# wangxb29/PPST

Hardware: AMD Instinct MI355X
Metric: 512x512 portrait swaps/sec/GPU (higher is better)
Workload: dtype bf16x3 (fp32 split into hi+lo bf16, 3 MFMA passes, fp32 accumulate); 1 GPU; simple_swapping 512x512 batch=8 per GPU, generator+encoders forward only (BASELINE configs[1]); image_parallel=1 batch per rank, no data-path collective

## Files before the change

include/ppst_hip.h:

```cpp
#ifndef PPST_HIP_H
#define PPST_HIP_H

#include <stddef.h>
#include <stdint.h>

#ifdef __cplusplus
extern "C" {
#endif

#define PPST_OK 0
#define PPST_EINVAL (-1)
#define PPST_EUNSUPPORTED (-2)
#define PPST_ENULL (-3)

enum { PPST_F32 = 0, PPST_F16 = 1, PPST_BF16 = 2, PPST_F64 = 3  };

enum { PPST_PAD_ZERO = 0, PPST_PAD_REFLECT = 1, PPST_PAD_REPLICATE = 2 };

enum { PPST_ACT_NONE = 0, PPST_ACT_LRELU = 1 , PPST_ACT_PRELU = 2 };

#define PPST_ABI_VERSION 3
int ppst_version(void);

#define PPST_ST_F32 0
// ... 67 lines not shown
int ppst_upscale_weight(const void* w, void* out, int cout, int cin, float scale, void* stream);
int ppst_dgrad_s2d_stack_weight(const void* w, void* out, int cout, int cin, void* stream);
int ppst_depth_to_space_st(const void* x, void* y, int B, int th, int tw, int oh, int ow, int C, int st, void* stream);

#define PPST_KSPLIT_SCRATCH_BYTES ((size_t)256 * 512 * 128 * 4)
#define PPST_KSPLIT_FLAG_WORDS 4096

typedef struct ppst_conv_args {
  const void* x;
  const void* wpack;
  const void* steps;
  void* y;
  const void* bias;
  const void* noise;
  const void* prelu;
  void* stats;
  const void* residual;
  float noise_weight;
  float out_scale;
  int32_t B, in_h, in_w, in_ld;
  int32_t out_h, out_w, out_ld, cout;
  int32_t nsteps, n_groups;
  int32_t pad_mode;
  int32_t in_off_y, in_off_x;
  int32_t out_sy, out_sx;
  int32_t act;
  int32_t precision;
  int32_t res_ld;
  int32_t tile_h, tile_w;
  int32_t halo;
  int32_t bn;
  const void* in_scale_shift;
  const void* in_prelu;
  int32_t in_c, in_act;
  int32_t flop_steps;
  int32_t tile_rows;
  int32_t a_slots;
  int32_t early_a;
  int32_t variant;
  int32_t in_presplit;
  int32_t dual_b;
  int32_t io_st;
  int32_t k64;
  const void* in_res;
  int32_t in_res_ld;
  int32_t ksplit;
  const int32_t* ksplit_starts;
  void* ksplit_scratch;
  unsigned* ksplit_flags;
  uint32_t ksplit_epoch;
} ppst_conv_args;

int ppst_conv2d_mfma(const ppst_conv_args* a, void* stream);
int64_t ppst_conv_pack_wino_bytes(int cout, int cin);
int ppst_conv_pack_wino(const void* w, int64_t sn, int64_t sc, int64_t sy, int64_t sx, float scale, int cout, int cin,
                        void* out, void* stream);
int ppst_presplit(const void* x, void* y, int64_t npix, int C, int x_ld, int y_ld, void* stream);
int ppst_has_experiments(void);
int ppst_conv2d_f32(const ppst_conv_args* a, const void* w, int64_t sn, int64_t sc, int64_t sy, int64_t sx, float wscale,
                    const int32_t* src_c, const int32_t* src_ky, const int32_t* src_kx, void* stream);
int ppst_conv_tiles(int tile_h, int tile_w, int tile_rows);

int ppst_conv1x1_small_cin(const void* x, const void* w, const void* bias, void* y,
                           int64_t npix, int cin, int in_ld, int cout, float wscale,
                           int act, void* stream);
int ppst_conv1x1_small_cin_st(const void* x, const void* w, const void* bias, void* y,
                              int64_t npix, int cin, int in_ld, int cout, float wscale,
                              int act, int y_st , void* stream);
int ppst_conv1x1_small_cout(const void* x, const void* w, const void* bias, void* y,
                            int64_t npix, int cin, int cout, float wscale, void* stream);
int ppst_conv1x1_small_cout_st(const void* x, const void* w, const void* bias, void* y,
                               int64_t npix, int cin, int cout, float wscale, int x_st , void* stream);
int ppst_torgb_apply_st(const void* x, const void* scale_shift, const void* res, int res_ld, float out_scale, const void* w,
                        const void* bias, void* y, int B, int H, int W, int cin, float wscale, int x_st, void* stream);

int ppst_in_stats(const void* x, void* partial, int B, int H, int W, int C, int ld,
                  int rep_pad, int* n_partials, void* stream);
int ppst_in_finalize(const void* partial, int n_partials, const void* style,
                     int style_ld ,
                     const void* post_bias ,
                     void* scale_shift , int B, int C, double count,
                     float eps, void* stream);
int ppst_affine_act(const void* x, const void* scale_shift, const void* res,
                    const void* res_scale_shift , void* y,
                    int B, int64_t hw, int C, int x_ld, int res_ld, int y_ld,
                    int act , const void* prelu,
                    float out_scale,
                    int res_up2_w ,
                    void* stream);
int ppst_affine_act_st(const void* x, const void* scale_shift, const void* res, const void* res_scale_shift, void* y,
                       int B, int64_t hw, int C, int x_ld, int res_ld, int y_ld, int act, const void* prelu,
                       float out_scale, int res_up2_w, int x_st, int y_st, void* stream);
int ppst_affine_act_stats(const void* x, const void* scale_shift, const void* res,
                          const void* res_scale_shift, void* y, void* partial,
                          int B, int H, int W, int C, int x_ld, int res_ld, int y_ld,
                          int act, const void* prelu, float out_scale, int rep_pad,
                          int res_up2 , void* stream);
int ppst_upsample_nearest2(const void* x, void* y, int B, int H, int W, int C, void* stream);
int ppst_upsample_nearest2_st(const void* x, void* y, int B, int H, int W, int C, int st, void* stream);

int64_t ppst_gap_gmp_ws(int B, int64_t hw, int C);
int ppst_gap_gmp(const void* x, const void* mask, void* out, void* ws, int B, int H, int W,
                 int C, int ld, void* stream);
int ppst_gap_gmp_st(const void* x, const void* mask, void* out, void* ws, int B, int H, int W,
                    int C, int ld, int x_st, void* stream);
int ppst_avgpool(const void* x, void* y, int B, int H, int W, int C, int x_ld, int f,
// ... 158 lines not shown
```

ppst_amd/_lib.py:

```python
import ctypes
import os

import torch

HERE = os.path.dirname(os.path.abspath(__file__))
LIB_PATH = os.environ.get("PPST_HIP_LIB") or os.path.join(HERE, "libppst_hip.so")

if not os.path.exists(LIB_PATH):
    raise ImportError(
        "ppst_amd: %s is missing -- build it with `python -m ppst_amd.build` "
        "(hipcc --offload-arch=gfx950). There is no CPU fallback." % LIB_PATH)

lib = ctypes.CDLL(LIB_PATH)

vp, i32, i64, f32, f64 = ctypes.c_void_p, ctypes.c_int, ctypes.c_int64, ctypes.c_float, ctypes.c_double


class PackJob(ctypes.Structure):
    _fields_ = [("w", vp), ("sn", i64), ("sc", i64), ("sy", i64), ("sx", i64), ("src_c", vp), ("src_ky", vp), ("src_kx", vp),
                ("out", vp), ("total", i64), ("block0", i64), ("scale", f32), ("cout", i32), ("bn", i32), ("nsteps", i32),
                ("n_groups", i32), ("x3", i32), ("f16", i32), ("nblocks", i32), ("dual", i32)]


class UpscaleJob(ctypes.Structure):
    _fields_ = [("w", vp), ("out", vp), ("total", i64), ("block0", i64), ("scale", f32), ("cout", i32), ("cin", i32), ("nblocks", i32)]


class ConvArgs(ctypes.Structure):
    _fields_ = [
        ("x", vp), ("wpack", vp), ("steps", vp), ("y", vp), ("bias", vp), ("noise", vp),
        ("prelu", vp), ("stats", vp), ("residual", vp),
        ("noise_weight", f32), ("out_scale", f32),
        ("B", i32), ("in_h", i32), ("in_w", i32), ("in_ld", i32),
        ("out_h", i32), ("out_w", i32), ("out_ld", i32), ("cout", i32),
        ("nsteps", i32), ("n_groups", i32), ("pad_mode", i32),
        ("in_off_y", i32), ("in_off_x", i32), ("out_sy", i32), ("out_sx", i32),
        ("act", i32), ("precision", i32), ("res_ld", i32), ("tile_h", i32), ("tile_w", i32),
        ("halo", i32), ("bn", i32), ("in_scale_shift", vp), ("in_prelu", vp), ("in_c", i32), ("in_act", i32),
        ("flop_steps", i32), ("tile_rows", i32), ("a_slots", i32), ("early_a", i32), ("variant", i32), ("in_presplit", i32), ("dual_b", i32), ("io_st", i32), ("k64", i32),
        ("in_res", vp), ("in_res_ld", i32), ("ksplit", i32), ("ksplit_starts", vp),
        ("ksplit_scratch", vp), ("ksplit_flags", vp), ("ksplit_epoch", ctypes.c_uint32),
    ]


_SIGS = {
    "ppst_version": (i32, []),
    "ppst_guided_filter_tune": (i32, [i32, i32]),
    "ppst_upfirdn2d": (i32, [vp, vp, vp] + [i32] * 14 + [i32, vp]),
    "ppst_blur_nhwc": (i32, [vp, vp, vp] + [i32] * 10 + [vp, i32, vp]),
    "ppst_blur_nhwc_st": (i32, [vp, vp, vp] + [i32] * 10 + [vp, i32, i32, vp]),
    "ppst_fused_bias_act": (i32, [vp, vp, vp, vp, i64, i32, i32, i32, i32, f32, f32, i32, vp]),
    "ppst_nchw_to_nhwc": (i32, [vp, vp, i32, i32, i32, i32, vp]),
    "ppst_nhwc_to_nchw": (i32, [vp, vp, i32, i32, i32, i32, vp]),
    "ppst_conv_pack": (i32, [vp, i64, i64, i64, i64, f32, i32, i32, vp, vp, vp, i32, i32, i32, vp, vp]),
    "ppst_conv_pack_k64": (i32, [vp, i64, i64, i64, i64, f32, i32, i32, vp, vp, vp, i32, i32, i32, i32, vp, vp]),
    "ppst_conv_pack_up9_bytes": (i64, [i32, i32]),
    "ppst_conv_pack_up9": (i32, [vp, i64, i64, i64, i64, f32, i32, i32, vp, vp]),
    "ppst_conv_pack_wino_bytes": (i64, [i32, i32]),
    "ppst_conv_pack_wino": (i32, [vp, i64, i64, i64, i64, f32, i32, i32, vp, vp]),
    "ppst_conv_pack_dual": (i32, [vp, i64, i64, i64, i64, f32, i32, vp, vp, vp, i32, i32, i32, vp, vp]),
    "ppst_upscale_weight": (i32, [vp, vp, i32, i32, f32, vp]),
    "ppst_dgrad_s2d_stack_weight": (i32, [vp, vp, i32, i32, vp]),
    "ppst_depth_to_space_st": (i32, [vp, vp, i32, i32, i32, i32, i32, i32, i32, vp]),
    "ppst_pack_job_blocks": (i32, [i64]),
    "ppst_conv_pack_batch": (i32, [vp, i32, i32, vp]),
    "ppst_upscale_weight_batch": (i32, [vp, i32, i32, vp]),
    "ppst_conv2d_mfma": (i32, [ctypes.POINTER(ConvArgs), vp]),
    "ppst_has_experiments": (i32, []),
    "ppst_presplit": (i32, [vp, vp, i64, i32, i32, i32, vp]),
    "ppst_conv2d_f32": (i32, [ctypes.POINTER(ConvArgs), vp, i64, i64, i64, i64, f32, vp, vp, vp, vp]),
    "ppst_conv_tiles": (i32, [i32, i32, i32]),
    "ppst_conv1x1_small_cin": (i32, [vp, vp, vp, vp, i64, i32, i32, i32, f32, i32, vp]),
    "ppst_conv1x1_small_cin_st": (i32, [vp, vp, vp, vp, i64, i32, i32, i32, f32, i32, i32, vp]),
    "ppst_conv1x1_small_cout": (i32, [vp, vp, vp, vp, i64, i32, i32, f32, vp]),
    "ppst_conv1x1_small_cout_st": (i32, [vp, vp, vp, vp, i64, i32, i32, f32, i32, vp]),
    "ppst_torgb_apply_st": (i32, [vp, vp, vp, i32, f32, vp, vp, vp, i32, i32, i32, i32, f32, i32, vp]),
    "ppst_in_stats": (i32, [vp, vp, i32, i32, i32, i32, i32, i32, ctypes.POINTER(i32), vp]),
    "ppst_in_finalize": (i32, [vp, i32, vp, i32, vp, vp, i32, i32, f64, f32, vp]),
    "ppst_affine_act": (i32, [vp, vp, vp, vp, vp, i32, i64, i32, i32, i32, i32, i32, vp, f32, i32, vp]),
    "ppst_affine_act_st": (i32, [vp, vp, vp, vp, vp, i32, i64, i32, i32, i32, i32, i32, vp, f32, i32, i32, i32, vp]),
    "ppst_affine_act_stats": (i32, [vp, vp, vp, vp, vp, vp, i32, i32, i32, i32, i32, i32, i32, i32, vp, f32, i32, i32, vp]),
    "ppst_upsample_nearest2": (i32, [vp, vp, i32, i32, i32, i32, vp]),
    "ppst_upsample_nearest2_st": (i32, [vp, vp, i32, i32, i32, i32, i32, vp]),
    "ppst_gap_gmp_ws": (i64, [i32, i64, i32]),
    "ppst_gap_gmp": (i32, [vp, vp, vp, vp, i32, i32, i32, i32, i32, vp]),
    "ppst_gap_gmp_st": (i32, [vp, vp, vp, vp, i32, i32, i32, i32, i32, i32, vp]),
    "ppst_avgpool": (i32, [vp, vp, i32, i32, i32, i32, i32, i32, i32, vp]),
    "ppst_bilinear": (i32, [vp, vp, i32, i32, i32, i32, i32, i32, i32, i32, vp]),
    "ppst_head_tail": (i32, [vp, vp, vp, vp, vp] + [i32] * 10 + [vp]),
    "ppst_maxpool2": (i32, [vp, vp, i32, i32, i32, i32, vp]),
    "ppst_linear": (i32, [vp, vp, vp, vp, i32, i32, i32, f32, f32, i32, i32, vp]),
    "ppst_l2norm_rows": (i32, [vp, vp, i32, i32, f32, i32, vp]),
    "ppst_lerp": (i32, [vp, vp, vp, i64, f32, vp]),
    "ppst_spatial_modulation": (i32, [vp, vp, vp, vp, i32, i64, i32, vp]),
    "ppst_spatial_modulation_st": (i32, [vp, vp, vp, vp, i32, i64, i32, i32, vp]),
    "ppst_rselfcorr": (i32, [vp, vp, i32, i32, i32, i32, i32, vp]),
    "ppst_corr_prep": (i32, [vp, vp, i32, i32, i32, i32, vp]),
    "ppst_gemm_nt_f32": (i32, [vp, vp, vp, i32, i32, i32, i32, f32, vp]),
    "ppst_gemm_nn_f32": (i32, [vp, vp, vp, i32, i32, i32, i32, i32, i32, vp]),
    "ppst_unfold_rows": (i32, [vp, vp, i32, i32, i32, i32, i32, vp]),
    "ppst_unfold_rows_bwd": (i32, [vp, vp, i32, i32, i32, i32, i32, vp]),
    "ppst_gemm_nt_split": (i32, [vp, vp, vp, i32, i32, i32, i32, f32, i32, vp]),
    "ppst_gemm_nn_split": (i32, [vp, vp, vp, i32, i32, i32, i32, i32, i32, i32, vp]),
    "ppst_softmax_rows": (i32, [vp, i64, i32, f32, vp]),
    "ppst_unfold_patches": (i32, [vp, vp, i32, i32, i32, i32, i32, vp]),
    "ppst_fold_patches": (i32, [vp, vp, i32, i32, i32, i32, i32, vp]),
    "ppst_tensor2im_u8": (i32, [vp, vp, i32, i32, i32, i32, vp]),
    "ppst_resample_u8": (i32, [vp, vp, i32, i32, i32, i32, i32, i32, vp, vp, i32, vp]),
    "ppst_u8_to_tensor": (i32, [vp, vp, i32, i32, i32, i32, f32, f32, vp]),
    "ppst_guided_filter_ws": (i64, [i32, i32, i32]),
    "ppst_guided_filter": (i32, [vp, vp, vp, vp, i32, i32, i32, i32, f32, vp, vp]),
    "ppst_smooth_local_affine_ws": (i64, [i32, i32, i32]),
    "ppst_smooth_local_affine": (i32, [vp, vp, vp, vp, vp, i32, i32, i32, i32, i32, f32, f32, vp]),
    "ppst_conv_wgrad_f32": (i32, [vp, vp, vp, vp, vp] + [i32] * 11 + [vp]),
    "ppst_conv_wgrad_bf16x3": (i32, [vp, vp, vp, vp, vp] + [i32] * 11 + [vp]),
    "ppst_conv_wgrad_tr": (i32, [vp, vp, vp, vp, vp, vp, i32, i32, i32, i32, i32, i32, i32, i32, i32, i32, i32, vp]),
    "ppst_conv_wgrad_tr2": (i32, [vp, vp, vp, vp, vp, vp, i32, i32, i32, i32, i32, i32, i32, i32, i32, i32, i32, i32, i32, i32, i32, vp]),
    "ppst_wgrad_scatter": (i32, [vp, vp, vp, vp, vp, i64, i64, i64, i64, i32, i32, i32, f32, i32, vp, vp, i32, i32, vp]),
    "ppst_wgrad_small_cin_ws": (i64, [i64, i32, i32]),
    "ppst_wgrad_small_cin": (i32, [vp, vp, vp, vp, i64, i32, i32, i32, f32, i32, vp]),
# ... 77 lines not shown
```

ppst_amd/build.py:

```python
import os
import subprocess
import sys
from concurrent.futures import ThreadPoolExecutor

HERE = os.path.dirname(os.path.abspath(__file__))
CSRC = os.path.join(HERE, "csrc")
OBJ = os.path.join(HERE, "csrc", "_obj")
LIB = os.path.join(HERE, "libppst_hip.so")
EXPERIMENTS = os.environ.get("PPST_EXPERIMENTS") == "1"
SOURCES = ["upfirdn2d.hip", "fused_bias_act.hip", "elementwise.hip", "linear.hip", "conv_mfma.hip", "conv_mfma2.hip", "conv1x1.hip", "conv_wino.hip", "conv_f32.hip",
           "corr.hip", "guided_filter.hip", "train.hip", "train_g.hip", "imageio.hip", "smooth_filter.hip"] + (["conv_ksplit.hip"] if EXPERIMENTS else [])
FLAGS = ["--offload-arch=gfx950", "-O3", "-fPIC", "-std=c++17", "-Wno-unused-result"] + (["-DPPST_EXPERIMENTS"] if EXPERIMENTS else [])
FILE_FLAGS = {"conv_wino.hip": ["-fno-slp-vectorize"]}
MODE_STAMP = os.path.join(HERE, ".libmode")


def _hipcc():
    for c in (os.environ.get("HIPCC"), "/opt/rocm/bin/hipcc", "hipcc"):
        if c and (os.path.isabs(c) and os.path.exists(c) or not os.path.isabs(c)):
            return c
    return "hipcc"


HEADERS = [os.path.join(CSRC, "common.h"), os.path.join(CSRC, "rscl_common.h"), os.path.join(HERE, "..", "include", "ppst_hip.h")]


def _stale(target, deps):
    return not os.path.exists(target) or any(os.path.getmtime(d) > os.path.getmtime(target) for d in deps)


def _mode():
    return "experiments" if EXPERIMENTS else "production"


def _lib_flavour():
    try:
        return open(MODE_STAMP).read().strip()
    except OSError:
        pass
    if not os.path.exists(LIB):
        return None
    try:
        return "experiments" if b"conv_ksplit_kernel" in open(LIB, "rb").read() else "production"
    except OSError:
        return None


def _mode_changed():
    have = _lib_flavour()
    if have is None:
        return os.path.exists(LIB)
    return have != _mode()


def needs_build():
    return (_mode_changed() or _stale(LIB, [os.path.join(CSRC, s) for s in SOURCES] + HEADERS) or
            any(_stale(os.path.join(OBJ, s.replace(".hip", ".o")), [os.path.join(CSRC, s)]) for s in SOURCES if os.path.isdir(OBJ)))


def build(force=False, verbose=True):
    if not force and not needs_build():
        return LIB
    os.makedirs(OBJ, exist_ok=True)
# ... 30 lines not shown
```

ppst_amd/networks/base_network.py:

```python
import math

import torch
from torch import nn

from .. import ops, weights

SQRT2 = math.sqrt(2.0)
INV_SQRT2 = 1.0 / SQRT2


class _Node(nn.Module):
    """parameter container (no behaviour)."""


def to_nhwc(x):
    if x.dim() != 4:
        raise RuntimeError("expected a 4-D NCHW tensor")
    v = x.permute(0, 2, 3, 1)
    if v.is_contiguous():
        ops._chk(v, "input")
        return v
    return ops.nchw_to_nhwc(x)


# ... 58 lines not shown
        val = build()
        self._cache[key] = (ver, val)
        return val

    def plan(self, wname, kind="conv", scale=1.0):
        w = self.p(wname)
        return self.cached(("plan", wname, kind), [w], lambda: ops.ConvPlan(w, kind=kind, scale=scale))

    def refresh_plans(self):
        plans, keep = [], {}
        for key, (ver, val) in self._cache.items():
            if isinstance(key, tuple) and key and key[0] == "plan" and isinstance(val, ops.ConvPlan) and val.precision != 2 \
                    and val.wparam.data_ptr() == self.p(key[1]).data_ptr():
                plans.append(val)
                keep[key] = (ver, val)
        self._cache.clear()
        if not plans:
            return
        sig = tuple((id(pl), tuple(sorted(map(str, pl._packs)))) for pl in plans)
        hit = self.__dict__.get("_repack")
        if hit is not None and hit[0] == sig:
            ops.run_repack(hit[1])
        else:
            self.__dict__["_repack"] = (sig, ops.repack_plans(plans), plans)
        self._cache.update(keep)

    def print_architecture(self, verbose=False):
        n = sum(p.numel() for p in self.parameters())
        print("[Network %s] Total number of parameters : %.3f M" % (type(self).__name__, n / 1e6))

    def from_rgb(self, x, p, out_dtype=torch.float32):
        w = self.p(p + "Conv.weight")
        return ops.conv1x1_small_cin(x, w, self.p(p + "Act.bias"), 1.0 / math.sqrt(w.shape[1]), ops.ACT_LRELU, out_dtype=out_dtype)

    def _norm_act(self, y, st, count, act_bias=None, act=ops.ACT_NONE, **kw):
        ss = ops.in_finalize(st, count, post_bias=act_bias)
        return ops.affine_act(y, ss, act=act, **kw), ss

    def res_block(self, x, p, blur_pad_mode, norm):
        B, H, W, cin = x.shape
        k = self.p(p + "conv2.Blur.kernel")
        ks = k.shape[0]
        w1, w2, ws = self.p(p + "conv1.Conv.weight"), self.p(p + "conv2.Conv.weight"), self.p(p + "skip.Conv.weight")
        sc1 = 1.0 / math.sqrt(cin * 9)
        scs = 1.0 / math.sqrt(cin)
        conv_pad = ops.PAD_REFLECT if blur_pad_mode == ops.PAD_REFLECT else ops.PAD_ZERO
        pad_c = (ks - 2) + 2
        pad_s = (ks - 2) + 0
        xs, _ = ops.blur_nhwc(x, self.p(p + "skip.Blur.kernel"), (pad_s + 1) // 2, pad_s // 2, ops.PAD_ZERO, down=2)
        if not norm:
            y1 = self.plan(p + "conv1.Conv.weight", scale=sc1)(x, bias=self.p(p + "conv1.Act.bias"), act=ops.ACT_LRELU,
                                                                pad_mode=conv_pad)
            skip = self.plan(p + "skip.Conv.weight", scale=scs)(xs)
            xb, bhw = ops.blur_nhwc(y1, k, (pad_c + 1) // 2, pad_c // 2, blur_pad_mode, s2d=True)
            ohw = ((bhw[0] - 3) // 2 + 1, (bhw[1] - 3) // 2 + 1)
            return self.plan(p + "conv2.Conv.weight", "s2d", sc1)(
                xb, bias=self.p(p + "conv2.Act.bias"), act=ops.ACT_LRELU, residual=skip, res_after_act=True,
                out_scale=INV_SQRT2, out_hw=ohw)
        y1, st1 = self.plan(p + "conv1.Conv.weight", scale=sc1)(x, stats=True, pad_mode=conv_pad)
        ss1 = ops.in_finalize(st1, H * W, post_bias=self.p(p + "conv1.Act.bias"))
        ys, sts = self.plan(p + "skip.Conv.weight", scale=scs)(xs, stats=True)
        xb, bhw = ops.blur_nhwc(y1, k, (pad_c + 1) // 2, pad_c // 2, blur_pad_mode, s2d=True, in_ss=ss1, in_act=ops.ACT_LRELU)
        ohw = ((bhw[0] - 3) // 2 + 1, (bhw[1] - 3) // 2 + 1)
        y2, st2 = self.plan(p + "conv2.Conv.weight", "s2d", sc1)(xb, stats=True, out_hw=ohw)
        cnt = ohw[0] * ohw[1]
        ss_s = ops.in_finalize(sts, cnt)
        ss2 = ops.in_finalize(st2, cnt, post_bias=self.p(p + "conv2.Act.bias"))
        return ops.affine_act(y2, ss2, res=ys, res_scale_shift=ss_s, act=ops.ACT_LRELU, out_scale=INV_SQRT2)
```

ppst_amd/ops.py:

```python
import ctypes
import math
import os
import threading

import torch

from . import _lib
from ._lib import lib, check

PAD_ZERO, PAD_REFLECT, PAD_REPLICATE = 0, 1, 2
ACT_NONE, ACT_LRELU, ACT_PRELU = 0, 1, 2
RES_BEFORE_ACT = 1 << 8

PRECISION = {"value": 0}
TILE_ROWS = {"value": 16}
CONV_VARIANT = {"value": 2}
DUAL_CONVT = {"value": True, "min_blocks": 32}
UP9 = {"value": True, "min_blocks": 64, "min_fill": 0.85}
DIRECT_MAX = {"cout": 64, "nsteps": 40, "cout3x3": 64}
WGRAD_SPLIT = {"blocks": 1024, "min_tiles": 4}
WGRAD_X3 = {"value": True}
STREAM_1X1 = {"value": True}
KSPLIT = {"value": os.environ.get("PPST_KSPLIT", "1") != "0", "max_blocks": 256, "min_steps": 16, "variants": (0, 2, 10)}
KSPLIT_SCRATCH_BYTES = 256 * 512 * 128 * 4
KSPLIT_FLAG_WORDS = 4096
KSPLIT_128 = {"value": False, "min_blocks": 32}
TALL_TILE_128 = {"value": False, "min_blocks": 32}
TALL_TILE_SINGLE = {"value": True, "min_blocks": 64}
K64 = {"value": True}
TILE24_128 = {"value": False, "min_blocks": 32, "max_waste": 0.04}
TWO_BLOCK_128 = {"value": False}
TWO_BLOCK_8ROW = {"value": False, "min_blocks": 64}
BATCH_AWARE = {"value": False, "fill": 192}


class batch_aware:

    def __enter__(self):
        self.prev = BATCH_AWARE["value"]
        BATCH_AWARE["value"] = True

    def __exit__(self, *exc):
        BATCH_AWARE["value"] = self.prev
WINO = {"value": True, "min_blocks": 16, "fill": 0, "ksplit_fill": 64}
FUSE_TAIL = {"value": os.environ.get("PPST_FUSE_TAIL", "1") != "0", "torgb": os.environ.get("PPST_FUSE_TORGB", "0") == "1"}
FAT_MIN_BLOCKS = 32


EXPERIMENTS = bool(lib.ppst_has_experiments())


def _need_experiments(what):
    if not EXPERIMENTS:
        raise RuntimeError("%s is an experiment kernel: rebuild the library with PPST_EXPERIMENTS=1 (python -m ppst_amd.build)" % what)


def set_precision(p):
    assert p in (0, 1, 2, 3, 4)
    if p == 4:
        _need_experiments("precision 4 (two-pass fp16)")
    PRECISION["value"] = p


_raw_stream = getattr(torch._C, "_cuda_getCurrentRawStream", None)
_cur_device = getattr(torch._C, "_cuda_getDevice", None)


def _stream():
    if _raw_stream is not None and _cur_device is not None:
        return ctypes.c_void_p(_raw_stream(_cur_device()))
    return ctypes.c_void_p(torch.cuda.current_stream().cuda_stream)


def _chk(t, name="tensor"):
    if t is None:
        return
    if not isinstance(t, torch.Tensor) or not t.is_cuda:
        raise RuntimeError("%s must be a CUDA (HIP) tensor" % name)
    if t.dtype != torch.float32:
        raise RuntimeError("%s must be float32, got %s" % (name, t.dtype))


def _p(t):
    return None if t is None else ctypes.c_void_p(t.data_ptr())


_ST = {torch.float32: 0, torch.float16: 1, torch.bfloat16: 2}
HALF_STORE = {"value": os.environ.get("PPST_HALF_STORE", "1") != "0"}


def act_dtype():
    if HALF_STORE["value"] and not torch.is_grad_enabled():
        return {1: torch.bfloat16, 3: torch.float16}.get(PRECISION["value"], torch.float32)
    return torch.float32


TRAIN_HALF = {"value": os.environ.get("PPST_TRAIN_HALF", "1") != "0"}

# ... 617 lines not shown
                                                   else self.pack_for(bn))
            steps_t = self.steps_up9 if up9 else self.steps_dual if dual else self.steps
        a.x, a.wpack, a.steps, a.y = _p(x), _p(wp), _p(steps_t), _p(out)
        a.k64 = 1 if k64 else 0
        a.variant = variant
        a.dual_b = 1 if dual else 0
        a.bias, a.noise, a.prelu, a.stats = _p(bias), _p(noise), _p(prelu), _p(st)
        a.residual = _p(residual)
        a.res_ld = _nhwc_ld(residual, "residual", half_ok=True) if residual is not None else 0
        a.io_st = _ST[x.dtype]
        a.noise_weight, a.out_scale = float(noise_weight), float(out_scale)
        a.B, a.in_h, a.in_w, a.in_ld = B, H, W, in_ld
        a.out_h, a.out_w, a.out_ld, a.cout = oh, ow, out_ld, self.cout
        a.nsteps, a.n_groups, a.pad_mode = (self.nsteps // 2 if k64 else self.nsteps), (1 if up9 else 2 if dual else self.n_groups), pad_mode
        a.in_off_y = a.in_off_x = 0
        a.out_sy = a.out_sx = osy
        a.act, a.precision = act | (0x100 if res_after_act else 0), self.precision
        a.tile_h, a.tile_w, a.halo, a.bn, a.tile_rows = th, tw, self.halo, bn, rows
        _chk(in_ss, "in_ss"); _chk(in_prelu, "in_prelu")
        a.in_scale_shift, a.in_prelu, a.in_act = _p(in_ss), _p(in_prelu), in_act
        a.in_c = in_ss.shape[1] if in_ss is not None else 0
        if in_res is not None:
            if variant != 4 or in_ss is None or self.precision != 0 or x.dtype != torch.float32:
                raise RuntimeError("in_res needs a 1x1 plan on the streaming kernel (ops.STREAM_1X1), in_ss, precision 0 and fp32 storage")
            if tuple(in_res.shape) != tuple(x.shape):
                raise RuntimeError("in_res must have the conv input's shape %s, got %s" % (tuple(x.shape), tuple(in_res.shape)))
            a.in_res, a.in_res_ld = _p(in_res), _nhwc_ld(in_res, "in_res")
        a.flop_steps = self.flop_steps
        a.a_slots = min(3, self.chunks_per_group)
        a.early_a = self.early_a
        if presplit:
            _need_experiments("pre-split conv input")
            if variant != 0 or bn != 128 or in_ss is not None or self.nsteps // max(1, self.chunks_per_group) < 4:
                raise RuntimeError("pre-split input: tile kernel (bn 128) plans with chunks of >= 4 steps and no in_ss only")
            a.in_presplit = 1
        ks_S, ks_cuts = self._ksplit(variant, a, self.precision == 2) if (KSPLIT["value"] and BATCH_AWARE["value"]) else (0, None)
        stream = _stream()
        if ks_S:
            ks_arr = (ctypes.c_int32 * (ks_S + 1))(*ks_cuts)
            a.ksplit, a.ksplit_starts = ks_S, ctypes.cast(ks_arr, ctypes.c_void_p)
            a.ksplit_scratch, a.ksplit_flags, a.ksplit_epoch = _ksplit_next(stream)
        if self.precision == 2:
            sn, sc, sy, sx = self.wstrides
            c_, ky_, kx_ = self.src_dev
            check(lib.ppst_conv2d_f32(ctypes.byref(a), _p(self.wsrc), sn, sc, sy, sx, self.scale, _p(c_), _p(ky_), _p(kx_), stream),
                  "ppst_conv2d_f32")
        else:
            check(lib.ppst_conv2d_mfma(ctypes.byref(a), stream), "ppst_conv2d_mfma")
        if stats:
            return out, st
        return out


class _KsWorkspace:
    __slots__ = ("scratch", "flags", "ptrs", "launches")

    def __init__(self):
        self.scratch = torch.empty(KSPLIT_SCRATCH_BYTES, dtype=torch.uint8, device="cuda")
        self.flags = torch.zeros(KSPLIT_FLAG_WORDS, dtype=torch.int32, device="cuda")
        self.ptrs = self.scratch.data_ptr(), self.flags.data_ptr()
        self.launches = 0


_ks_ws = {}
_ks_lock = threading.Lock()


def _ks_key(stream):
    return (_cur_device() if _cur_device is not None else torch.cuda.current_device()), stream.value


def _ksplit_next(stream):
    key = _ks_key(stream)
    with _ks_lock:
        ws = _ks_ws.get(key)
        if ws is None:
            ws = _ks_ws[key] = _KsWorkspace()
        ws.launches += 1
        epoch = (ws.launches - 1) % 0xFFFFFFFF + 1
    return ws.ptrs + (epoch,)


def ksplit_launches():
    ws = _ks_ws.get(_ks_key(_stream()))
    return ws.launches if ws is not None else 0


def ksplit_check():
    ws = _ks_ws.get(_ks_key(_stream()))
    if ws is None:
        torch.cuda.current_stream().synchronize()
        return True
    marker = ws.flags[KSPLIT_FLAG_WORDS - 1:]
    if marker.item() == 0:
        return True
    marker.zero_()
    return False


def _ksplit_choice(blocks, chunk_starts, max_blocks, min_steps, max_s=8):
    nsteps = chunk_starts[-1]
    for S in (8, 4, 2):
        if S > max_s or blocks * S > max_blocks or (S - 1) * blocks > 256 or len(chunk_starts) - 1 < S:
            continue
        cuts = [0]
        for i in range(1, S):
# ... 950 lines not shown
```

Before: 159.6 swaps/s (all GPUs).

## Fuse blur + stride-2 s2d conv into one down-sampling kernel

Adds a HIP kernel that stages the raw input tile into shared memory, optionally applies instance-norm scale/shift and leaky ReLU, runs the blur filter per parity phase, splits the result to bf16 hi/lo, and feeds it straight into 3-pass MFMA for the stride-2 conv. The epilogue handles bias, activation, residual and stats. The down-sampling residual blocks with reflect padding and cin<=32 now use it instead of a separate blur_nhwc pass plus conv. This removes the intermediate blurred-tensor write and read, at the cost of redundant blur work per cout block and extra shared-memory pressure.

```diff
diff --git a/include/ppst_hip.h b/include/ppst_hip.h
--- a/include/ppst_hip.h
+++ b/include/ppst_hip.h
@@ -143,6 +143,8 @@
 } ppst_conv_args;
 
 int ppst_conv2d_mfma(const ppst_conv_args* a, void* stream);
+int ppst_conv_down_blur(const ppst_conv_args* conv, const void* blur_k, int ksize, int pad0, int pad1, int pad_mode,
+                        const void* in_scale_shift, int in_act, int in_h, int in_w, void* stream);
 int64_t ppst_conv_pack_wino_bytes(int cout, int cin);
 int ppst_conv_pack_wino(const void* w, int64_t sn, int64_t sc, int64_t sy, int64_t sx, float scale, int cout, int cin,
                         void* out, void* stream);
diff --git a/ppst_amd/_lib.py b/ppst_amd/_lib.py
--- a/ppst_amd/_lib.py
+++ b/ppst_amd/_lib.py
@@ -66,6 +66,7 @@
     "ppst_conv_pack_batch": (i32, [vp, i32, i32, vp]),
     "ppst_upscale_weight_batch": (i32, [vp, i32, i32, vp]),
     "ppst_conv2d_mfma": (i32, [ctypes.POINTER(ConvArgs), vp]),
+    "ppst_conv_down_blur": (i32, [ctypes.POINTER(ConvArgs), vp, i32, i32, i32, i32, vp, i32, i32, i32, vp]),
     "ppst_has_experiments": (i32, []),
     "ppst_presplit": (i32, [vp, vp, i64, i32, i32, i32, vp]),
     "ppst_conv2d_f32": (i32, [ctypes.POINTER(ConvArgs), vp, i64, i64, i64, i64, f32, vp, vp, vp, vp]),
diff --git a/ppst_amd/build.py b/ppst_amd/build.py
--- a/ppst_amd/build.py
+++ b/ppst_amd/build.py
@@ -8,7 +8,7 @@
 OBJ = os.path.join(HERE, "csrc", "_obj")
 LIB = os.path.join(HERE, "libppst_hip.so")
 EXPERIMENTS = os.environ.get("PPST_EXPERIMENTS") == "1"
-SOURCES = ["upfirdn2d.hip", "fused_bias_act.hip", "elementwise.hip", "linear.hip", "conv_mfma.hip", "conv_mfma2.hip", "conv1x1.hip", "conv_wino.hip", "conv_f32.hip",
+SOURCES = ["upfirdn2d.hip", "fused_bias_act.hip", "elementwise.hip", "linear.hip", "conv_mfma.hip", "conv_mfma2.hip", "conv1x1.hip", "conv_wino.hip", "conv_f32.hip", "conv_down.hip",
            "corr.hip", "guided_filter.hip", "train.hip", "train_g.hip", "imageio.hip", "smooth_filter.hip"] + (["conv_ksplit.hip"] if EXPERIMENTS else [])
 FLAGS = ["--offload-arch=gfx950", "-O3", "-fPIC", "-std=c++17", "-Wno-unused-result"] + (["-DPPST_EXPERIMENTS"] if EXPERIMENTS else [])
 FILE_FLAGS = {"conv_wino.hip": ["-fno-slp-vectorize"]}
diff --git a/ppst_amd/csrc/conv_down.hip b/ppst_amd/csrc/conv_down.hip
--- /dev/null
+++ b/ppst_amd/csrc/conv_down.hip
@@ -0,0 +1,283 @@
+#include "common.h"
+
+struct DownKArgs {
+  const float* x;
+  const unsigned char* wpack;
+  const int4* steps;
+  float* y;
+  const float* bias;
+  float* stats;
+  const float* residual;
+  const float* in_ss;
+  const float* blur_k;
+  float out_scale;
+  int B, in_h, in_w, in_ld, cin, out_h, out_w, out_ld, cout, res_ld, nsteps, bn, act, res_mode, in_act, pad_mode, pad0;
+  int tiles_y, tiles_x;
+};
+
+__device__ __forceinline__ int cd_reflect(int i, int n) {
+  if (i < 0) i = -i;
+  if (i >= n) i = 2 * (n - 1) - i;
+  return i < 0 ? 0 : (i >= n ? n - 1 : i);
+}
+
+template <int KS, bool INSS>
+__global__ __launch_bounds__(256, 2) void conv_down_blur_kernel(DownKArgs a) {
+  constexpr int TH = 4, TW = 16, NT = 256;
+  constexpr int RH = 2 * TH + KS, RC = 2 * TW + KS;
+  constexpr int ODD = 19, RWP = ODD + RC / 2;
+  constexpr int RAW_BYTES = RH * RWP * 128;
+  constexpr int PW = TW + 1, PP = (TH + 1) * PW;
+  constexpr int PLANE = 1600;
+  constexpr int A_BYTES = 8 * PLANE;
+  constexpr int EPI_TILE = 16 * 68;
+  static_assert(PLANE >= PP * 16 && PLANE % 256 == 64, "plane pitch");
+  static_assert(RAW_BYTES >= 4 * EPI_TILE * 4 + 4 * 64 * 2 * 4, "the epilogue lives in the raw tile");
+  __shared__ __attribute__((aligned(1024))) unsigned char smem[RAW_BYTES + A_BYTES];
+  float* const raw = (float*)smem;
+  unsigned char* const smA = smem + RAW_BYTES;
+
+  const int nwg = gridDim.x;
+  int wid;
+  {
+    int id = blockIdx.x, q = nwg >> 3, r = nwg & 7, xcd = id & 7;
+    wid = (xcd < r ? xcd * (q + 1) : r * (q + 1) + (xcd - r) * q) + (id >> 3);
+  }
+  const int tiles = a.tiles_y * a.tiles_x;
+  const int m_count = a.B * tiles;
+  const int n64 = wid / m_count;
+  int midx = wid - n64 * m_count;
+  const int b = midx / tiles;
+  midx -= b * tiles;
+  const int tyi = midx / a.tiles_x, txi = midx - tyi * a.tiles_x;
+  const int ty0 = tyi * TH, tx0 = txi * TW;
+
+  const int tid = threadIdx.x, lane = tid & 63, wave = __builtin_amdgcn_readfirstlane(tid >> 6);
+  const int r16 = lane & 15, g = lane >> 4;
+
+  float kf[KS * KS];
+#pragma unroll
+  for (int i = 0; i < KS * KS; ++i) kf[i] = a.blur_k[KS * KS - 1 - i];
+
+  const int nb64 = a.bn >> 6;
+  const unsigned char* wblob = a.wpack + ((int64_t)(n64 / nb64) * a.nsteps) * (int64_t)(a.bn * 128) + (n64 % nb64) * 1024;
+  const int bplane = a.bn * 16;
+  const float* xb = a.x + (int64_t)b * a.in_h * a.in_w * a.in_ld;
+
+  constexpr int R_ITEMS = RH * RC * 8, R_IT = (R_ITEMS + NT - 1) / NT;
+  const int q = tid & 7;
+  auto stage_raw = [&](int c0) {
+    float4 rv[R_IT];
+    unsigned okm = 0;
+#pragma unroll
+    for (int it = 0; it < R_IT; ++it) {
+      const int i = tid + it * NT;
+      rv[it] = make_float4(0.f, 0.f, 0.f, 0.f);
+      if (i < R_ITEMS) {
+        const int px = i >> 3, r = px / RC, c = px - r * RC;
+        int iy = 2 * ty0 - a.pad0 + r, ix = 2 * tx0 - a.pad0 + c;
+        if (a.pad_mode == PPST_PAD_REFLECT) { iy = cd_reflect(iy, a.in_h); ix = cd_reflect(ix, a.in_w); }
+        if (iy >= 0 && iy < a.in_h && ix >= 0 && ix < a.in_w) {
+          rv[it] = *(const float4*)(xb + ((int64_t)iy * a.in_w + ix) * a.in_ld + c0 + q * 4);
+          okm |= 1u << it;
+        }
+      }
+    }
+    float4 sa = make_float4(1.f, 1.f, 1.f, 1.f), sb = make_float4(0.f, 0.f, 0.f, 0.f);
+    if (INSS) {
+      const float4* qp = (const float4*)(a.in_ss + ((int64_t)b * a.cin + c0 + q * 4) * 2);
+      const float4 q0 = qp[0], q1 = qp[1];
+      sa = make_float4(q0.x, q0.z, q1.x, q1.z); sb = make_float4(q0.y, q0.w, q1.y, q1.w);
+    }
+#pragma unroll
+    for (int it = 0; it < R_IT; ++it) {
+      const int i = tid + it * NT;
+      if (i < R_ITEMS) {
+        const int px = i >> 3, r = px / RC, c = px - r * RC;
+        float4 v = rv[it];
+        if (INSS && ((okm >> it) & 1)) {
+          v.x = __builtin_fmaf(sa.x, v.x, sb.x); v.y = __builtin_fmaf(sa.y, v.y, sb.y);
+          v.z = __builtin_fmaf(sa.z, v.z, sb.z); v.w = __builtin_fmaf(sa.w, v.w, sb.w);
+          if (a.in_act == PPST_ACT_LRELU) {
+            v.x = (v.x > 0.f ? v.x : v.x * 0.2f) * 1.41421356237309515f; v.y = (v.y > 0.f ? v.y : v.y * 0.2f) * 1.41421356237309515f;
+            v.z = (v.z > 0.f ? v.z : v.z * 0.2f) * 1.41421356237309515f; v.w = (v.w > 0.f ? v.w : v.w * 0.2f) * 1.41421356237309515f;
+          }
+        }
+        *(float4*)(raw + (r * RWP + (c >> 1) + (c & 1) * ODD) * 32 + q * 4) = v;
+      }
+    }
+  };
+
+  auto blur_phase = [&](int py, int px) {
+    for (int i = tid; i < PP * 8; i += NT) {
+      const int p = i >> 3, yy = p / PW, xx = p - yy * PW;
+      const int by = 2 * yy + py, bx = 2 * xx + px;
+      if (by > 2 * TH || bx > 2 * TW) continue;
+      float4 acc = make_float4(0.f, 0.f, 0.f, 0.f);
+#pragma unroll
+      for (int ry = 0; ry < KS; ++ry)
+#pragma unroll
+        for (int j = 0; j < KS; ++j) {
+          const int c = bx + j;
+          const float4 v = *(const float4*)(raw + ((by + ry) * RWP + (c >> 1) + (c & 1) * ODD) * 32 + q * 4);
+          const float f = kf[ry * KS + j];
+          acc.x = __builtin_fmaf(v.x, f, acc.x); acc.y = __builtin_fmaf(v.y, f, acc.y);
+          acc.z = __builtin_fmaf(v.z, f, acc.z); acc.w = __builtin_fmaf(v.w, f, acc.w);
+        }
+      uint2 hv, lv;
+      split_bf16x4(acc, hv, lv);
+      const int off = (q >> 1) * PLANE + p * 16 + (q & 1) * 8;
+      *(uint2*)(smA + off) = hv;
+      *(uint2*)(smA + 4 * PLANE + off) = lv;
+    }
+  };
+
+  f32x4 acc[4];
+#pragma unroll
+  for (int j = 0; j < 4; ++j) acc[j] = (f32x4){0.f, 0.f, 0.f, 0.f};
+
+  auto ld_b = [&](int s, bf16x8 (&dst)[8]) {
+    const unsigned char* src = wblob + (int64_t)s * (a.bn * 128) + g * bplane + r16 * 16;
+#pragma unroll
+    for (int nt = 0; nt < 4; ++nt) {
+      dst[nt] = *(const bf16x8*)(src + nt * 256);
+      dst[4 + nt] = *(const bf16x8*)(src + 4 * bplane + nt * 256);
+    }
+  };
+  const int nst = a.nsteps;
+  int4 d = a.steps[0];
+  bf16x8 b0[8], b1[8];
+  ld_b(0, b0);
+#define DOWN_STEP(s_, bc, bn_)                                                                        \
+  {                                                                                                   \
+    if ((s_) + 1 < nst) ld_b((s_) + 1, bn_);                                                          \
+    if (d.w & 1) {                                               \
+      const int phase = d.x / a.cin, c0 = d.x - phase * a.cin;                                        \
+      __syncthreads();                              \
+      if ((s_) == 0 || a.cin > 32) {                                                                  \
+        stage_raw(c0);                                                                                \
+        __syncthreads();                                                                              \
+      }                                                                                               \
+      blur_phase(phase >> 1, phase & 1);                                                              \
+      __syncthreads();                                                                                \
+    }                                                                                                 \
+    const unsigned char* Ab = smA + g * PLANE + ((wave + d.y) * PW + d.z + r16) * 16;                 \
+    const bf16x8 ah = *(const bf16x8*)Ab, al = *(const bf16x8*)(Ab + 4 * PLANE);                      \
+    _Pragma("unroll") for (int nt = 0; nt < 4; ++nt) {                                                \
+      acc[nt] = __builtin_amdgcn_mfma_f32_16x16x32_bf16(al, bc[nt], acc[nt], 0, 0, 0);                \
+      acc[nt] = __builtin_amdgcn_mfma_f32_16x16x32_bf16(ah, bc[4 + nt], acc[nt], 0, 0, 0);            \
+      acc[nt] = __builtin_amdgcn_mfma_f32_16x16x32_bf16(ah, bc[nt], acc[nt], 0, 0, 0);                \
+    }                                                                                                 \
+    d = a.steps[(s_) + 1];                                             \
+  }
+  for (int s = 0; s < nst; s += 2) {
+    DOWN_STEP(s, b0, b1)
+    DOWN_STEP(s + 1, b1, b0)
+  }
+#undef DOWN_STEP
+  __syncthreads();
+
+  float* tw = (float*)raw + wave * EPI_TILE;
+  float* red = (float*)raw + 4 * EPI_TILE;
+#pragma unroll
+  for (int nt = 0; nt < 4; ++nt)
+#pragma unroll
+    for (int j = 0; j < 4; ++j) tw[(g * 4 + j) * 68 + nt * 16 + r16] = acc[nt][j];
+  __builtin_amdgcn_s_waitcnt(0xC07F);
+  __builtin_amdgcn_wave_barrier();
+  {
+#pragma clang fp contract(off)
+    const int f16 = lane & 15, prow = lane >> 4;
+    const int n0 = n64 * 64 + f16 * 4;
+    const int oy = ty0 + wave;
+    float4 bv = make_float4(0.f, 0.f, 0.f, 0.f);
+    if (a.bias) bv = *(const float4*)(a.bias + n0);
+    float4 s1 = make_float4(0.f, 0.f, 0.f, 0.f), s2 = make_float4(0.f, 0.f, 0.f, 0.f);
+    const float nz = 0.f;
+#pragma unroll
+    for (int it = 0; it < 4; ++it) {
+      const int p = it * 4 + prow, ox = tx0 + p;
+      const float4 v = *(const float4*)(tw + p * 68 + f16 * 4);
+      if (oy < a.out_h && ox < a.out_w) {
+        const int64_t pix = ((int64_t)b * a.out_h + oy) * a.out_w + ox;
+        float4 rv = make_float4(0.f, 0.f, 0.f, 0.f);
+        if (a.res_mode) rv = *(const float4*)(a.residual + pix * a.res_ld + n0);
+        float o[4] = {v.x + bv.x + nz, v.y + bv.y + nz, v.z + bv.z + nz, v.w + bv.w + nz};
+        const float r4[4] = {rv.x, rv.y, rv.z, rv.w};
+#pragma unroll
+        for (int c = 0; c < 4; ++c) {
+          float t = o[c];
+          if (a.res_mode == 1) t += r4[c];
+          if (a.act == PPST_ACT_LRELU) t = (t > 0.f ? t : t * 0.2f) * 1.41421356237309515f;
+          if (a.res_mode == 2) t += r4[c];
+          o[c] = t * a.out_scale;
+        }
+        *(float4*)(a.y + pix * a.out_ld + n0) = make_float4(o[0], o[1], o[2], o[3]);
+        s1.x += o[0]; s1.y += o[1]; s1.z += o[2]; s1.w += o[3];
+        s2.x += o[0] * o[0]; s2.y += o[1] * o[1]; s2.z += o[2] * o[2]; s2.w += o[3] * o[3];
+      }
+    }
+    if (a.stats) {
+#pragma unroll
+      for (int o = 16; o < 64; o <<= 1) {
+        s1.x += __shfl_xor(s1.x, o, 64); s1.y += __shfl_xor(s1.y, o, 64); s1.z += __shfl_xor(s1.z, o, 64); s1.w += __shfl_xor(s1.w, o, 64);
+        s2.x += __shfl_xor(s2.x, o, 64); s2.y += __shfl_xor(s2.y, o, 64); s2.z += __shfl_xor(s2.z, o, 64); s2.w += __shfl_xor(s2.w, o, 64);
+      }
+      if (prow == 0) {
+        float* r = red + (wave * 64 + f16 * 4) * 2;
+        r[0] = s1.x; r[1] = s2.x; r[2] = s1.y; r[3] = s2.y; r[4] = s1.z; r[5] = s2.z; r[6] = s1.w; r[7] = s2.w;
+      }
+    }
+  }
+  if (a.stats) {
+    __syncthreads();
+    if (tid < 64) {
+      float s1 = 0.f, s2 = 0.f;
+#pragma unroll
+      for (int w = 0; w < 4; ++w) { s1 += red[(w * 64 + tid) * 2]; s2 += red[(w * 64 + tid) * 2 + 1]; }
+      float* o = a.stats + ((((int64_t)b * tiles) + tyi * a.tiles_x + txi) * a.cout + n64 * 64 + tid) * 2;
+      o[0] = s1;
+      o[1] = s2;
+    }
+  }
+}
+
+extern "C" int ppst_conv_down_blur(const ppst_conv_args* a, const void* blur_k, int ksize, int pad0, int pad1, int pad_mode,
+                                   const void* in_scale_shift, int in_act, int in_h, int in_w, void* stream) {
+  if (!a) return PPST_ENULL;
+  const int act = a->act & 0xff;
+  if (a->io_st != PPST_ST_F32 || a->precision != 0 || a->in_c <= 0 || a->in_c % 32 || a->cout <= 0 || a->cout % 64 || a->ksplit ||
+      (ksize != 3 && ksize != 4) || a->B < 0 || in_h <= 0 || in_w <= 0 || pad0 < 0 || pad1 < 0 ||
+      (pad_mode != PPST_PAD_ZERO && pad_mode != PPST_PAD_REFLECT) || (in_act != PPST_ACT_NONE && in_act != PPST_ACT_LRELU) ||
+      (act != PPST_ACT_NONE && act != PPST_ACT_LRELU) || a->noise || a->in_res || a->in_presplit || a->k64 || a->dual_b ||
+      a->n_groups != 1 || (a->bn != 64 && a->bn != 128) || a->cout % a->bn || a->nsteps != 10 * (a->in_c / 32) ||
+      a->in_ld < a->in_c || a->in_ld % 4 || a->out_ld < a->cout || a->out_ld % 4 || (a->residual && (a->res_ld < a->cout || a->res_ld % 4)) ||
+      (pad_mode == PPST_PAD_REFLECT && (pad0 >= in_h || pad0 >= in_w || pad1 >= in_h || pad1 >= in_w)))
+    return PPST_EINVAL;
+  const int bh = in_h + pad0 + pad1 - ksize + 1, bw = in_w + pad0 + pad1 - ksize + 1;
+  if (bh < 3 || bw < 3 || a->out_h != (bh - 3) / 2 + 1 || a->out_w != (bw - 3) / 2 + 1) return PPST_EINVAL;
+  if ((int64_t)in_h * in_w * a->in_ld * 4 > 0x7fffffff || (int64_t)a->out_h * a->out_w * a->out_ld * 4 > 0x7fffffff) return PPST_EINVAL;
+  if (a->B == 0) return PPST_OK;
+  if (!a->x || !a->wpack || !a->steps || !a->y || !blur_k) return PPST_ENULL;
+  DownKArgs k;
+  k.x = (const float*)a->x; k.wpack = (const unsigned char*)a->wpack; k.steps = (const int4*)a->steps; k.y = (float*)a->y;
+  k.bias = (const float*)a->bias; k.stats = (float*)a->stats; k.residual = (const float*)a->residual;
+  k.in_ss = (const float*)in_scale_shift; k.blur_k = (const float*)blur_k; k.out_scale = a->out_scale;
+  k.B = a->B; k.in_h = in_h; k.in_w = in_w; k.in_ld = a->in_ld; k.cin = a->in_c; k.out_h = a->out_h; k.out_w = a->out_w;
+  k.out_ld = a->out_ld; k.cout = a->cout; k.res_ld = a->res_ld; k.nsteps = a->nsteps; k.bn = a->bn; k.act = act;
+  k.res_mode = a->residual ? (((a->act >> 8) & 1) ? 2 : 1) : 0;
+  k.in_act = in_act; k.pad_mode = pad_mode; k.pad0 = pad0;
+  k.tiles_y = cdiv(a->out_h, 4); k.tiles_x = cdiv(a->out_w, 16);
+  const int64_t blocks = (int64_t)(a->cout / 64) * a->B * k.tiles_y * k.tiles_x;
+  if (blocks > 0x7fffffff) return PPST_EINVAL;
+  hipStream_t st = as_stream(stream);
+  const dim3 grid((unsigned)blocks), blk(256);
+  if (ksize == 3) {
+    if (k.in_ss) PPST_LAUNCH((conv_down_blur_kernel<3, true>), grid, blk, 0, st, k);
+    else PPST_LAUNCH((conv_down_blur_kernel<3, false>), grid, blk, 0, st, k);
+  } else {
+    if (k.in_ss) PPST_LAUNCH((conv_down_blur_kernel<4, true>), grid, blk, 0, st, k);
+    else PPST_LAUNCH((conv_down_blur_kernel<4, false>), grid, blk, 0, st, k);
+  }
+  return PPST_LAUNCH_CHECK();
+}
diff --git a/ppst_amd/networks/base_network.py b/ppst_amd/networks/base_network.py
--- a/ppst_amd/networks/base_network.py
+++ b/ppst_amd/networks/base_network.py
@@ -134,6 +134,10 @@
             y1 = self.plan(p + "conv1.Conv.weight", scale=sc1)(x, bias=self.p(p + "conv1.Act.bias"), act=ops.ACT_LRELU,
                                                                 pad_mode=conv_pad)
             skip = self.plan(p + "skip.Conv.weight", scale=scs)(xs)
+            pl2 = self.plan(p + "conv2.Conv.weight", "s2d", sc1)
+            if blur_pad_mode == ops.PAD_REFLECT and ops.conv_down_blur_ok(pl2, y1):
+                return ops.conv_down_blur(pl2, y1, k, (pad_c + 1) // 2, pad_c // 2, blur_pad_mode, bias=self.p(p + "conv2.Act.bias"),
+                                          act=ops.ACT_LRELU, residual=skip, res_after_act=True, out_scale=INV_SQRT2)
             xb, bhw = ops.blur_nhwc(y1, k, (pad_c + 1) // 2, pad_c // 2, blur_pad_mode, s2d=True)
             ohw = ((bhw[0] - 3) // 2 + 1, (bhw[1] - 3) // 2 + 1)
             return self.plan(p + "conv2.Conv.weight", "s2d", sc1)(
@@ -142,9 +146,15 @@
         y1, st1 = self.plan(p + "conv1.Conv.weight", scale=sc1)(x, stats=True, pad_mode=conv_pad)
         ss1 = ops.in_finalize(st1, H * W, post_bias=self.p(p + "conv1.Act.bias"))
         ys, sts = self.plan(p + "skip.Conv.weight", scale=scs)(xs, stats=True)
-        xb, bhw = ops.blur_nhwc(y1, k, (pad_c + 1) // 2, pad_c // 2, blur_pad_mode, s2d=True, in_ss=ss1, in_act=ops.ACT_LRELU)
-        ohw = ((bhw[0] - 3) // 2 + 1, (bhw[1] - 3) // 2 + 1)
-        y2, st2 = self.plan(p + "conv2.Conv.weight", "s2d", sc1)(xb, stats=True, out_hw=ohw)
+        pl2 = self.plan(p + "conv2.Conv.weight", "s2d", sc1)
+        if blur_pad_mode == ops.PAD_REFLECT and ops.conv_down_blur_ok(pl2, y1):
+            y2, st2 = ops.conv_down_blur(pl2, y1, k, (pad_c + 1) // 2, pad_c // 2, blur_pad_mode, in_ss=ss1, in_act=ops.ACT_LRELU,
+                                         stats=True)
+            ohw = tuple(y2.shape[1:3])
+        else:
+            xb, bhw = ops.blur_nhwc(y1, k, (pad_c + 1) // 2, pad_c // 2, blur_pad_mode, s2d=True, in_ss=ss1, in_act=ops.ACT_LRELU)
+            ohw = ((bhw[0] - 3) // 2 + 1, (bhw[1] - 3) // 2 + 1)
+            y2, st2 = pl2(xb, stats=True, out_hw=ohw)
         cnt = ohw[0] * ohw[1]
         ss_s = ops.in_finalize(sts, cnt)
         ss2 = ops.in_finalize(st2, cnt, post_bias=self.p(p + "conv2.Act.bias"))
diff --git a/ppst_amd/ops.py b/ppst_amd/ops.py
--- a/ppst_amd/ops.py
+++ b/ppst_amd/ops.py
@@ -44,6 +44,7 @@
         BATCH_AWARE["value"] = self.prev
 WINO = {"value": True, "min_blocks": 16, "fill": 0, "ksplit_fill": 64}
 FUSE_TAIL = {"value": os.environ.get("PPST_FUSE_TAIL", "1") != "0", "torgb": os.environ.get("PPST_FUSE_TORGB", "0") == "1"}
+FUSE_DOWN = {"value": os.environ.get("PPST_FUSE_DOWN", "1") != "0", "max_cin": 32}
 FAT_MIN_BLOCKS = 32
 
 
@@ -767,6 +768,44 @@
         return out
 
 
+def conv_down_blur_ok(plan, x):
+    return (FUSE_DOWN["value"] and plan.kind == "s2d" and plan.precision == 0 and x.dtype == torch.float32
+            and plan.cin % 32 == 0 and plan.cin <= FUSE_DOWN["max_cin"] and plan.cout % 64 == 0 and plan.cout % plan.bn == 0
+            and plan.nsteps == 10 * (plan.cin // 32))
+
+
+def conv_down_blur(plan, x, kernel, pad0, pad1, pad_mode=PAD_ZERO, in_ss=None, in_act=ACT_NONE, bias=None, act=ACT_NONE, stats=False,
+                   residual=None, res_after_act=False, out_scale=1.0):
+    in_ld = _nhwc_ld(x, "conv input")
+    B, H, W, C = x.shape
+    if plan.kind != "s2d" or plan.precision != 0 or x.dtype != torch.float32 or C != plan.cin:
+        raise RuntimeError("conv_down_blur needs an 's2d' plan of precision 0 and its fp32 input of %d channels" % plan.cin)
+    _chk(kernel, "kernel"); _chk(in_ss, "in_ss"); _chk(bias, "bias")
+    ks = kernel.shape[0]
+    if in_ss is not None and (tuple(in_ss.shape) != (B, C, 2) or not in_ss.is_contiguous()):
+        raise RuntimeError("in_ss must be a contiguous (B=%d, %d, 2) table, got %s" % (B, C, tuple(in_ss.shape)))
+    bh, bw = H + pad0 + pad1 - ks + 1, W + pad0 + pad1 - ks + 1
+    oh, ow = (bh - 3) // 2 + 1, (bw - 3) // 2 + 1
+    out = torch.empty((B, oh, ow, plan.cout), device=x.device, dtype=x.dtype)
+    if residual is not None and (tuple(residual.shape) != tuple(out.shape) or residual.dtype != x.dtype):
+        raise RuntimeError("residual must match the output %s, got %s" % (tuple(out.shape), tuple(residual.shape)))
+    st = None
+    if stats:
+        st = torch.empty((B, ((oh + 3) // 4) * ((ow + 15) // 16), plan.cout, 2), device=x.device, dtype=torch.float32)
+    a = _lib.ConvArgs()
+    a.x, a.wpack, a.steps, a.y = _p(x), _p(plan.pack_for(plan.bn)), _p(plan.steps), _p(out)
+    a.bias, a.stats, a.residual = _p(bias), _p(st), _p(residual)
+    a.res_ld = _nhwc_ld(residual, "residual") if residual is not None else 0
+    a.out_scale = float(out_scale)
+    a.B, a.in_ld, a.in_c = B, in_ld, C
+    a.out_h, a.out_w, a.out_ld, a.cout = oh, ow, plan.cout, plan.cout
+    a.nsteps, a.n_groups, a.bn = plan.nsteps, 1, plan.bn
+    a.act, a.precision = act | (0x100 if res_after_act else 0), plan.precision
+    check(lib.ppst_conv_down_blur(ctypes.byref(a), _p(kernel.contiguous()), ks, pad0, pad1, pad_mode, _p(in_ss), in_act, H, W,
+                                  _stream()), "ppst_conv_down_blur")
+    return (out, st) if stats else out
+
+
 class _KsWorkspace:
     __slots__ = ("scratch", "flags", "ptrs", "launches")
 
```

Result: no change. 160.2 swaps/s (all GPUs) (median of 6 runs) (+0.4%).
